# lazear/sage

Hardware: AMD Instinct MI355X
Metric: spectra/sec (whole node), fragment-index search-and-score, human tryptic narrow search (higher is better)
Workload: dtype f32

## Files before the change

include/sage_hip.h:

```cpp
#ifndef SAGE_HIP_H
#define SAGE_HIP_H

#include <stddef.h>
#include <stdint.h>

#ifdef __cplusplus
extern "C" {
#endif

#define SAGE_HIP_ABI_VERSION 6

enum {
    SAGE_HIP_OK = 0,
    SAGE_HIP_ERR_INVALID = 1,
    SAGE_HIP_ERR_NO_DEVICE = 2,
    SAGE_HIP_ERR_HIP = 3,
    SAGE_HIP_ERR_UNSUPPORTED = 4,
    SAGE_HIP_ERR_OOM = 5,
    SAGE_HIP_ERR_INTERNAL = 6
};

enum { SAGE_TOL_PPM = 0, SAGE_TOL_PCT = 1, SAGE_TOL_DA = 2 };
typedef struct SageTolerance {
    int32_t kind;
// ... 182 lines not shown
    float retry_ms;
    uint32_t n_tied;
    uint32_t n_ways;
} SageTiming;
int sage_hip_last_timing(const SageScorer* scorer, SageTiming* out);
int sage_hip_scorer_set_timing_interval(SageScorer* scorer, uint32_t every);

int sage_hip_host_alloc(uint64_t bytes, void** out);
void sage_hip_host_free(void* p);

int sage_hip_debug_phase_cycles(SageScorer* scorer, unsigned long long* out32);
int sage_hip_debug_prune_counters(SageScorer* scorer, unsigned long long* out4);
int sage_hip_debug_filter_counters(SageScorer* scorer, unsigned long long* out4);
int sage_hip_debug_heavy_counters(SageScorer* scorer, unsigned long long* out2);
int sage_hip_debug_heavy_routes(SageScorer* scorer, unsigned long long* out2);
int sage_hip_debug_handover_route(SageScorer* scorer, uint32_t* out);
#define SAGE_HIP_RESCORE_INST_CHIMERA 1u
#define SAGE_HIP_RESCORE_INST_KINDS2 2u
#define SAGE_HIP_RESCORE_INST_FAST 4u
#define SAGE_HIP_RESCORE_INST_ACC 8u
#define SAGE_HIP_RESCORE_INST_PROF 16u
#define SAGE_HIP_RESCORE_INST_BIG 32u
#define SAGE_HIP_RESCORE_INST_NONE 0xFFFFFFFFu
int sage_hip_debug_rescore_instance(SageScorer* scorer, uint32_t* out);

typedef struct SageDbLayout {
    uint64_t np, nf;
    uint32_t tile_shift, n_tiles, lut_stride;
    float lut_scale;
    uint32_t tile2_shift, n_tiles2, lut2_stride;
// ... 309 lines not shown
```

sage_amd/_lib.py:

```python
import ctypes as C
import os

import numpy as np

from . import build as _build

c_float_p = C.POINTER(C.c_float)
c_u8_p = C.POINTER(C.c_uint8)
c_u32_p = C.POINTER(C.c_uint32)
c_u64_p = C.POINTER(C.c_uint64)


class SageTolerance(C.Structure):
    _fields_ = [("kind", C.c_int32), ("lo", C.c_float), ("hi", C.c_float)]


class SageTheoretical(C.Structure):
    _fields_ = [("peptide_index", C.c_uint32), ("fragment_mz", C.c_float)]


class SageDbParams(C.Structure):
    _fields_ = [
        ("bucket_size", C.c_uint64),
        ("missed_cleavages", C.c_int32),
# ... 311 lines not shown
        "sage_hip_batch_upload_kinds": (C.c_int, [vp, C.POINTER(SageSpectrumBatch), c_u8_p, C.POINTER(vp)]),
        "sage_hip_batch_process_upload_kinds": (C.c_int, [vp, C.POINTER(SageRawBatch), c_u8_p, C.c_uint64, C.c_int, C.c_float,
                                                          C.c_uint32, C.POINTER(vp), c_u32_p]),
        "sage_hip_score_batch_kinds": (C.c_int, [vp, C.POINTER(SageSpectrumBatch), c_u8_p, vp, c_u32_p]),
        "sage_hip_score_resident": (C.c_int, [vp, vp, vp, c_u32_p]),
        "sage_hip_initial_hits": (C.c_int, [vp, vp, c_u64_p, C.c_uint32, c_u32_p, c_u64_p, c_u64_p]),
        "sage_hip_last_timing": (C.c_int, [vp, C.POINTER(SageTiming)]),
        "sage_hip_scorer_set_timing_interval": (C.c_int, [vp, C.c_uint32]),
        "sage_hip_annotate_resident": (C.c_int, [vp, vp, vp, c_u32_p, C.POINTER(SageFragments)]),
        "sage_hip_quick_score_resident": (C.c_int, [vp, vp, C.c_int, c_u8_p]),
        "sage_hip_debug_phase_cycles": (C.c_int, [vp, c_u64_p]),
        "sage_hip_debug_prune_counters": (C.c_int, [vp, c_u64_p]),
        "sage_hip_debug_filter_counters": (C.c_int, [vp, c_u64_p]),
        "sage_hip_debug_heavy_counters": (C.c_int, [vp, c_u64_p]),
        "sage_hip_debug_heavy_routes": (C.c_int, [vp, c_u64_p]),
        "sage_hip_debug_handover_route": (C.c_int, [vp, c_u32_p]),
        "sage_hip_debug_rescore_instance": (C.c_int, [vp, c_u32_p]),
        "sage_hip_debug_db_layout": (C.c_int, [vp, C.POINTER(SageDbLayout)]),
        "sage_hip_debug_db_table": (C.c_int, [vp, C.c_int, vp, C.c_uint64, c_u64_p]),
        "sage_hip_host_alloc": (C.c_int, [C.c_uint64, C.POINTER(vp)]),
        "sage_hip_host_free": (None, [vp]),
        "sage_hip_rescore": (C.c_int, [C.c_int, C.POINTER(SageRescoreInput), C.POINTER(SageRescoreOutput)]),
        "sage_hip_hostdb_competition_keys": (C.c_int, [vp, c_u32_p, C.c_uint64, c_u32_p, c_u32_p, c_u32_p, c_u32_p]),
        "sage_hip_predict_rt": (C.c_int, [C.c_int, C.POINTER(SageRtInput), C.POINTER(SageRtOutput)]),
        "sage_hip_hostdb_feature_peptides": (C.c_int, [vp, c_u32_p, C.c_uint64, c_u64_p, c_u8_p, c_float_p]),
        "sage_hip_mzml_read": (C.c_int, [C.c_char_p, C.c_uint32, C.c_int, C.POINTER(vp)]),
        "sage_hip_mzml_view": (C.c_int, [vp, C.POINTER(SageRawBatch)]),
        "sage_hip_mzml_check_searchable": (C.c_int, [vp]),
        "sage_hip_mzml_spectrum_id": (C.c_char_p, [vp, C.c_uint64]),
        "sage_hip_mzml_free": (None, [vp]),
# ... 39 lines not shown
    }
    for name, (res, args) in sig.items():
        fn = getattr(lib, name)
        fn.restype = res
        fn.argtypes = args
    _lib = lib
    return lib


EXPORTED_SYMBOLS = [
    "sage_hip_last_error", "sage_hip_abi_version", "sage_hip_hostdb_build", "sage_hip_hostdb_free",
    "sage_hip_hostdb_view", "sage_hip_hostdb_peptide_string", "sage_hip_hostdb_peptide_proteins",
    "sage_hip_hostdb_peptide_info", "sage_hip_process_ms2", "sage_hip_device_count", "sage_hip_db_create", "sage_hip_db_destroy",
    "sage_hip_db_device_bytes", "sage_hip_scorer_create", "sage_hip_scorer_destroy", "sage_hip_scorer_clone", "sage_hip_score_batch",
    "sage_hip_batch_upload", "sage_hip_batch_free", "sage_hip_batch_process_upload", "sage_hip_batch_download", "sage_hip_score_resident", "sage_hip_initial_hits",
    "sage_hip_last_timing", "sage_hip_scorer_set_timing_interval", "sage_hip_annotate_resident", "sage_hip_quick_score_resident", "sage_hip_debug_phase_cycles", "sage_hip_debug_prune_counters", "sage_hip_debug_filter_counters", "sage_hip_debug_heavy_counters", "sage_hip_debug_heavy_routes", "sage_hip_debug_handover_route", "sage_hip_debug_rescore_instance", "sage_hip_debug_db_layout", "sage_hip_debug_db_table", "sage_hip_host_alloc", "sage_hip_host_free",
    "sage_hip_rescore", "sage_hip_hostdb_competition_keys", "sage_hip_fasta_num_targets", "sage_hip_prefilter_chunk_size",
    "sage_hip_hostdb_build_chunk", "sage_hip_hostdb_merge_kept", "sage_hip_predict_rt", "sage_hip_hostdb_feature_peptides",
    "sage_hip_write_results", "sage_hip_mzml_read", "sage_hip_mzml_view", "sage_hip_mzml_check_searchable", "sage_hip_mzml_spectrum_id", "sage_hip_mzml_free",
    "sage_hip_lfq", "sage_hip_write_lfq", "sage_hip_mzml_read_sn", "sage_hip_mzml_ion_injection_time", "sage_hip_mzml_precursor_ref",
    "sage_hip_tmt", "sage_hip_write_tmt", "sage_hip_mgf_read", "sage_hip_mzml_isolation_kinds", "sage_hip_mzml_charge_zero",
    "sage_hip_parse_f32", "sage_hip_batch_upload_kinds", "sage_hip_batch_process_upload_kinds", "sage_hip_score_batch_kinds",
    "sage_hip_lfq_im", "sage_hip_mzml_mobility", "sage_hip_mzml_has_mobility",
    "sage_hip_protein_groups", "sage_hip_group_string", "sage_hip_group_strings_free", "sage_hip_group_graph_build",
    "sage_hip_group_graph_view", "sage_hip_group_graph_free", "sage_hip_hostdb_protein_name", "sage_hip_write_results_grouped",
    "sage_hip_hostdb_isomer_groups", "sage_hip_score_candidates_resident", "sage_hip_last_candidates_timing",
    "sage_hip_localise_resident", "sage_hip_ascore_from_counts", "sage_hip_last_localise_timing",
]


def check(rc):
# ... 8 lines not shown
```

sage_amd/csrc/capi.hip:

```cpp
#include <hip/hip_runtime.h>
#include <algorithm>
#include <atomic>
#include <cmath>
#include <chrono>
#include <cstring>
#include <memory>
#include <future>
#include <mutex>
#include <string>
#include <vector>

#include "crlog.h"
#include "device_types.h"
#define HIP_FAILED(e, what) fail(status_of(e), std::string(what) + ": " + hipGetErrorString(e))
#include "hip_host.h"
#include "host_db.hpp"

using namespace sagehip;

namespace {

thread_local std::string g_last_error;

int fail(int code, const std::string& msg) {
// ... 944 lines not shown
    d.list_cap = d.kmax * (std::max(n_iso, n_z) + 1);
    d.wcap = 1024;
    d.dbg_flags = 0;
    if (const char* e = getenv("SAGE_HIP_DEBUG_FLAGS")) d.dbg_flags = (uint32_t)atoi(e);
    s->hand_rows = (d.dbg_flags & 131072u) == 0u;
    d.prune_min = (d.dbg_flags & 4096u) ? 0u : d.min_matched_peaks;
    d.rescore_general = 0;
    if (const char* e = getenv("SAGE_HIP_RESCORE_GENERAL")) d.rescore_general = atoi(e) != 0 ? RESCORE_GENERAL_CHIMERA : 0u;
    {
        const DevDbView& v = db->view;
        bool kinds2 = v.n_kinds == 2u && v.ion_kinds[0] <= 2 && v.ion_kinds[1] > 2;
        if (const char* e = getenv("SAGE_HIP_RESCORE_KINDS_GENERAL")) kinds2 = kinds2 && atoi(e) == 0;
        if (!kinds2) d.rescore_general |= RESCORE_GENERAL_KINDS;
    }
    d.exact = 0;
    d.xcd_chunk = 1024;
    if (const char* e = getenv("SAGE_HIP_XCD_CHUNK")) d.xcd_chunk = (uint32_t)std::max(0, atoi(e));
    {
        const char* e = getenv("SAGE_HIP_SCHED_DESC");
        if (!e || atoi(e)) d.xcd_chunk |= 0x80000000u;
        s->sched_desc_forced = e != nullptr;
    }
    if (const char* e = getenv("SAGE_HIP_EXACT")) s->exact_always = atoi(e) != 0;
    if (const char* e = getenv("SAGE_HIP_FUSED")) s->fused = atoi(e) != 0;
    if (const char* e = getenv("SAGE_HIP_ONE_LANE")) s->two_lanes = atoi(e) == 0;
    if (const char* e = getenv("SAGE_HIP_SEARCH_LAG")) s->search_lag = (uint32_t)std::max(0, atoi(e));
    if (const char* e = getenv("SAGE_HIP_REPLAY_WAVE_MAX")) s->replay_split = (uint64_t)atoll(e) & 0xFFFFFFFFull;
    if (const char* e = getenv("SAGE_HIP_REPLAY_LANE_MAX")) s->replay_split |= (uint64_t)(uint32_t)atoll(e) << 32;
    if (const char* e = getenv("SAGE_HIP_ONE_LAUNCH")) s->one_launch = atoi(e) != 0;
#ifndef SAGE_HIP_EXPERIMENTS
    if (s->one_launch || s->fused || getenv("SAGE_HIP_SEARCH_LAG"))
        return fail(SAGE_HIP_ERR_UNSUPPORTED, "SAGE_HIP_ONE_LAUNCH / SAGE_HIP_FUSED / SAGE_HIP_SEARCH_LAG need a build with -DSAGE_HIP_EXPERIMENTS");
#endif
    if (const char* e = getenv("SAGE_HIP_NO_ZEROCOPY")) s->zero_copy = atoi(e) == 0;
    if (const char* e = getenv("SAGE_HIP_NO_FAST_TIES")) s->fast_ties = atoi(e) == 0;
// ... 613 lines not shown
    w.tile_shift = s->db->view.tile_shift;
    w.dbg = s->dbg.p;
    return w;
}

enum { MODE_SCORE = 0,
       MODE_EXACT = 1,
       MODE_FAST = 2 };

static int enqueue_compute(SageScorer* s, const DevBatchView& view_in, OutSet& o, bool with_rescore, int mode, hipStream_t st,
                           SageFeature* rec = nullptr, bool wide = true, uint32_t list_off = 0, uint32_t* count_buf = nullptr,
                           int lane = 0, int phase = 0, uint32_t widest = 0xFFFFFFFFu) {
    if (lane && wide) return fail(SAGE_HIP_ERR_INTERNAL, "large windows on the second working set");
    WorkSet& wset = lane ? s->ws2 : s->ws;
    DevScorer sc = s->dev;
    if (wide && !s->sched_desc_forced) sc.xcd_chunk &= 0x7FFFFFFFu;
    DevBatchView view = view_in;
    {
        const WindowKey mine = window_key(s);
        view.sched_win = view.sched && view.sched_stride == SCHED_RECORD_WINDOW && view.sched_key && std::memcmp(view.sched_key, &mine, sizeof mine) == 0;
    }
    if (!view.probe && (size_t)view.fzcap * view.pcap * 8 > 48 * 1024) view.probe = 1;
    if (!view.probe) {
        const int rc_pm = ensure_pm_frag(s->db);
        if (rc_pm != SAGE_HIP_OK) return rc_pm;
    }
    const bool production = mode == MODE_SCORE && with_rescore;
    const bool fused = s->fused && production;
    if (!production) wide = true;
    int rc = ensure_work(s, view.n, lane, wide, st);
    if (rc != SAGE_HIP_OK) return rc;
// ... 990 lines not shown
        for (uint32_t k = 0; k < 2; k++) out2[k] += all[b * DBG_PRUNE_WORDS + 8 + k];
    return SAGE_HIP_OK;
}

int sage_hip_debug_heavy_routes(SageScorer* s, unsigned long long* out2) {
    if (!s || !out2) return fail(SAGE_HIP_ERR_INVALID, "null argument");
    if (!s->dbg.p) return fail(SAGE_HIP_ERR_INVALID, "set SAGE_HIP_PHASE_CLOCKS=1 before creating the scorer");
    std::vector<unsigned long long> all((size_t)DBG_BLOCKS * DBG_PRUNE_WORDS);
    HIP_TRY(hipMemcpy(all.data(), s->dbg.p + (size_t)DBG_BLOCKS * 32, all.size() * 8, hipMemcpyDeviceToHost));
    out2[0] = out2[1] = 0;
    for (size_t b = 0; b < DBG_BLOCKS; b++)
        for (uint32_t k = 0; k < 2; k++) out2[k] += all[b * DBG_PRUNE_WORDS + 10 + k];
    return SAGE_HIP_OK;
}

int sage_hip_debug_handover_route(SageScorer* s, uint32_t* out) {
    if (!s || !out) return fail(SAGE_HIP_ERR_INVALID, "null argument");
    *out = s->last_hand ? 1u : 0u;
    return SAGE_HIP_OK;
}

int sage_hip_debug_rescore_instance(SageScorer* s, uint32_t* out) {
    if (!s || !out) return fail(SAGE_HIP_ERR_INVALID, "null argument");
    static_assert(RESCORE_INST_CHIMERA == SAGE_HIP_RESCORE_INST_CHIMERA && RESCORE_INST_KINDS2 == SAGE_HIP_RESCORE_INST_KINDS2 &&
                      RESCORE_INST_FAST == SAGE_HIP_RESCORE_INST_FAST && RESCORE_INST_ACC == SAGE_HIP_RESCORE_INST_ACC &&
                      RESCORE_INST_PROF == SAGE_HIP_RESCORE_INST_PROF && RESCORE_INST_BIG == SAGE_HIP_RESCORE_INST_BIG &&
                      RESCORE_INST_NONE == SAGE_HIP_RESCORE_INST_NONE,
                  "include/sage_hip.h names the bits of device_types.h");
    *out = s->last_rescore;
    return SAGE_HIP_OK;
// ... 114 lines not shown
```

sage_amd/csrc/core.h:

```cpp
#pragma once
#include <stdint.h>

#if defined(__HIPCC__)
#define SAGE_HD __host__ __device__ __forceinline__
#else
#define SAGE_HD inline
#endif

namespace sagecore {

constexpr float PROTON = 1.0072764f;
constexpr float NEUTRON = 1.00335f;

struct Tol {
    int kind;
    float lo, hi;
};

SAGE_HD void tol_bounds(const Tol& t, float center, float& out_lo, float& out_hi) {
    if (t.kind == 0) {
        float dlo = center * t.lo / 1000000.0f;
        float dhi = center * t.hi / 1000000.0f;
        out_lo = center + dlo;
        out_hi = center + dhi;
// ... 640 lines not shown
#ifndef SAGE_FLAT_MARGIN
#define SAGE_FLAT_MARGIN 1
#endif
constexpr uint32_t FLAT_MARGIN = SAGE_FLAT_MARGIN;
SAGE_HD uint32_t flat_route_bar(uint32_t total) { return (total + 63u) / 64u + FLAT_MARGIN; }
SAGE_HD bool flat_route_wins(uint32_t total, uint32_t longest) { return total != 0u && longest > flat_route_bar(total); }
SAGE_HD uint32_t flat_mask_word(uint32_t lo, uint32_t hi, uint32_t start) {
#if defined(__HIP_DEVICE_COMPILE__)
    return __builtin_amdgcn_alignbyte(hi, lo, start & 3u);
#else
    const uint32_t sh = (start & 3u) * 8u;
    return sh ? (lo >> sh) | (hi << (32u - sh)) : lo;
#endif
}

}
```

sage_amd/csrc/device_types.h:

```cpp
#pragma once
#include <stdint.h>

#include <string>

#include "../../include/sage_hip.h"
#include "core.h"

namespace sagehip {

struct DevDbView {
    const float* pep_mono;
    uint32_t np;
    const uint32_t* pep_lut;
    uint32_t pep_lut_bins;
    float pep_lut_inv_w;
    const SageTheoretical* pm_frag;
    const uint64_t* pm_off;
    const float* ions;
    const uint64_t* ion_off;
    const uint32_t* pep_info;
    const SageTheoretical* tm_frag;
    const uint32_t* tm_lut;
    uint32_t tile_shift;
    uint32_t n_tiles;
// ... 3 lines not shown
    const sagecore::LutWord* tm2_l1;
    const uint32_t* tm2_pos;
    uint32_t lut2_words;
    uint32_t tile2_shift;
    uint32_t n_tiles2;
    uint32_t lut2_stride;
    float lut2_scale;
    uint64_t nf;
    uint8_t ion_kinds[8];
    uint32_t n_kinds;
};

constexpr uint32_t TILE_SHIFT_MAX = 15;
__host__ __device__ inline size_t tm_lut_index(uint32_t t, uint32_t c, uint32_t lut_stride) { return (size_t)t * lut_stride + c; }

constexpr uint32_t DBG_BLOCKS = 4096, DBG_PRUNE_WORDS = 12;
constexpr size_t DBG_TOTAL_WORDS = (size_t)DBG_BLOCKS * (32 + DBG_PRUNE_WORDS);

struct DevScorer {
    sagecore::Tol precursor_tol, fragment_tol;
    sagecore::PbmReach pbm_reach;
    uint32_t min_matched_peaks;
    int min_isotope_err, max_isotope_err;
    uint32_t min_precursor_charge, max_precursor_charge;
    uint32_t override_precursor_charge;
    int max_fragment_charge;
    uint32_t chimera;
    uint32_t report_psms;
    uint32_t wide_window;
    int score_type;
    uint32_t kmax;
// ... 213 lines not shown
```

sage_amd/csrc/kernels.hip:

```cpp
#include <hip/hip_runtime.h>

#include <type_traits>

#include "crlog.h"
#include "device_types.h"

using namespace sagecore;

namespace sagehip {

namespace {

#ifndef SAGE_PRELIM_WAVES
#define SAGE_PRELIM_WAVES 5
#endif
#ifndef SAGE_RESCORE_WAVES
#define SAGE_RESCORE_WAVES 5
#endif
#ifndef SAGE_NARROW_WAVES
#define SAGE_NARROW_WAVES 5
#endif
#ifndef SAGE_PROBE_PER_LANE
#define SAGE_PROBE_PER_LANE 2
#endif
// ... 9 lines not shown
#ifndef SAGE_MARK_BLOCKS16
#define SAGE_MARK_BLOCKS16 40
#endif
#ifndef SAGE_COOP_MIN_HITS
#define SAGE_COOP_MIN_HITS 12
#endif
#ifndef SAGE_COOP_MAX_LANES
#define SAGE_COOP_MAX_LANES 2
#endif
#ifndef SAGE_CNT_MODE
#define SAGE_CNT_MODE 0
#endif
#ifndef SAGE_SCAN_SKIP
#define SAGE_SCAN_SKIP 1
#endif
#if SAGE_NARROW_WAVES
#define SAGE_NARROW_WAVES_ATTR __attribute__((amdgpu_waves_per_eu(SAGE_NARROW_WAVES, SAGE_NARROW_WAVES)))
#else
#define SAGE_NARROW_WAVES_ATTR
#endif
#if SAGE_PRELIM_WAVES
#define SAGE_PRELIM_WAVES_ATTR __attribute__((amdgpu_waves_per_eu(SAGE_PRELIM_WAVES, SAGE_PRELIM_WAVES)))
#else
#define SAGE_PRELIM_WAVES_ATTR
#endif
#if SAGE_RESCORE_WAVES
#define SAGE_RESCORE_WAVES_ATTR __attribute__((amdgpu_waves_per_eu(SAGE_RESCORE_WAVES, SAGE_RESCORE_WAVES)))
#else
#define SAGE_RESCORE_WAVES_ATTR
#endif

constexpr uint32_t WAVE = 64;
constexpr uint32_t NO_WINDOW = 0xFFFFFFFFu;
constexpr uint32_t FAST_TIE_WORDS = PBM_WORDS + PLUT_BINS;
constexpr uint32_t CNT_ROW_HEADER = 4;
constexpr uint32_t PROBE_BATCH_WORDS = SAGE_PROBE_PER_LANE * 64;
constexpr uint32_t PROBE_TCS_WORDS = PROBE_BATCH_WORDS <= 64 ? 64 : PROBE_BATCH_WORDS <= 128 ? 128 : PROBE_BATCH_WORDS <= 256 ? 256 : 512;
constexpr uint32_t PROBE_TABLE_WORDS = 4 * PROBE_BATCH_WORDS + PROBE_TCS_WORDS;

enum { DBG_PRUNE_CAND = 0, DBG_PRUNE_ITEMS = 1, DBG_PRUNE_EARLY = 2, DBG_PRUNE_MIXED = 3 };
enum { DBG_FILTER_FLAT_CHUNKS = 4, DBG_FILTER_FLAT_TRIPS = 5, DBG_FILTER_FLAT_WOULD = 6, DBG_FILTER_LANE_TRIPS = 7 };
enum { DBG_HEAVY_CHUNKS = 8, DBG_HEAVY_ITEMS = 9 };
enum { DBG_HEAVY_ONE_TRIP = 10, DBG_HEAVY_PER_CHARGE = 11 };
enum { DBG_NARROW_LUT = 26, DBG_NARROW_CELLS = 27, DBG_RESCORE = 28, DBG_TILE_LUT = 29, DBG_TILE_CELLS = 30, DBG_TILE_CAND = 31 };
struct PhaseClock {
    unsigned long long* slot;
    long long t;
    __device__ __forceinline__ void bytes(int which, unsigned long long n) {
        if (slot) atomicAdd(&slot[which - row_base], n);
    }
    int row_base;
    unsigned long long* prune;
    uint32_t pruned_here;
    __device__ __forceinline__ void pruned(uint64_t lanes, uint32_t items) {
        if (slot && lanes) {
            pruned_here += (uint32_t)__popcll(lanes);
            if ((threadIdx.x & 63u) == 0) {
                atomicAdd(&prune[DBG_PRUNE_CAND], (unsigned long long)__popcll(lanes));
// ... 9 lines not shown
                atomicAdd(&prune[DBG_FILTER_FLAT_WOULD], (unsigned long long)lane_trips);
            } else {
                atomicAdd(&prune[DBG_FILTER_LANE_TRIPS], (unsigned long long)lane_trips);
            }
        }
    }
    __device__ __forceinline__ void heavy(uint32_t items) {
        if (slot && (threadIdx.x & 63u) == 0) {
            atomicAdd(&prune[DBG_HEAVY_CHUNKS], 1ull);
            atomicAdd(&prune[DBG_HEAVY_ITEMS], (unsigned long long)items);
        }
    }
    __device__ __forceinline__ void heavy_route(bool one_trip) {
        if (slot && (threadIdx.x & 63u) == 0) atomicAdd(&prune[one_trip ? DBG_HEAVY_ONE_TRIP : DBG_HEAVY_PER_CHARGE], 1ull);
    }
    __device__ __forceinline__ void prune_outcome(bool left_early, bool any_pass) {
        if (slot && (threadIdx.x & 63u) == 0) {
            if (left_early) atomicAdd(&prune[DBG_PRUNE_EARLY], 1ull);
            else if (any_pass && pruned_here) atomicAdd(&prune[DBG_PRUNE_MIXED], 1ull);
        }
        pruned_here = 0;
    }
    __device__ __forceinline__ void start(unsigned long long* dbg, uint32_t blk, uint32_t kernel) {
        slot = dbg ? dbg + (size_t)(blk % DBG_BLOCKS) * 32 + kernel * 8 : nullptr;
        row_base = (int)kernel * 8;
        prune = dbg ? dbg + (size_t)DBG_BLOCKS * 32 + (size_t)(blk % DBG_BLOCKS) * DBG_PRUNE_WORDS : nullptr;
        pruned_here = 0;
        if (slot) t = clock64();
    }
    __device__ __forceinline__ void mark(int phase) {
// ... 5 lines not shown
    }
    __device__ __forceinline__ void rebase(uint32_t kernel) {
        if (slot) slot += (int)kernel * 8 - row_base;
        row_base = (int)kernel * 8;
    }
};

struct NoClock {
    static constexpr unsigned long long* slot = nullptr;
    __device__ __forceinline__ void bytes(int, unsigned long long) {}
    __device__ __forceinline__ void pruned(uint64_t, uint32_t) {}
    __device__ __forceinline__ void prune_outcome(bool, bool) {}
    __device__ __forceinline__ void filter_trips(bool, uint32_t, uint32_t) {}
    __device__ __forceinline__ void heavy(uint32_t) {}
    __device__ __forceinline__ void heavy_route(bool) {}
    __device__ __forceinline__ void start(unsigned long long*, uint32_t, uint32_t) {}
    __device__ __forceinline__ void mark(int) {}
    __device__ __forceinline__ void rebase(uint32_t) {}
};

__device__ __forceinline__ uint32_t lane_id() { return threadIdx.x & 63u; }

constexpr uint32_t N_XCD = 8;
__device__ __forceinline__ uint32_t xcd_position_fwd(uint32_t b, uint32_t n, uint32_t chunk) {
    if (chunk == 0) return b;
    const uint32_t group = N_XCD * chunk;
    if (b >= n / group * group) return b;
    const uint32_t x = b % N_XCD, i = b / N_XCD;
    return ((i / chunk) * N_XCD + x) * chunk + i % chunk;
}
__device__ __forceinline__ uint32_t xcd_position(uint32_t b, uint32_t n, uint32_t chunk) {
    const uint32_t p = xcd_position_fwd(b, n, chunk & 0x7FFFFFFFu);
    return (chunk & 0x80000000u) ? n - 1 - p : p;
}

__device__ __forceinline__ uint32_t fresh_zero() {
    uint32_t z;
    asm volatile("v_mov_b32 %0, 0" : "=v"(z));
    return z;
}
__device__ __forceinline__ uint32_t uni(uint32_t v) { return (uint32_t)__builtin_amdgcn_readfirstlane((int)v); }
__device__ __forceinline__ float unif(float v) { return __int_as_float(__builtin_amdgcn_readfirstlane(__float_as_int(v))); }
__device__ __forceinline__ uint64_t uni64(uint64_t v) { return ((uint64_t)uni((uint32_t)(v >> 32)) << 32) | uni((uint32_t)v); }

__device__ __forceinline__ uint32_t wave_sum_dpp(uint32_t v) {
    v += (uint32_t)__builtin_amdgcn_update_dpp(0, (int)v, 0xb1, 0xf, 0xf, false);
    v += (uint32_t)__builtin_amdgcn_update_dpp(0, (int)v, 0x4e, 0xf, 0xf, false);
    v += (uint32_t)__builtin_amdgcn_update_dpp(0, (int)v, 0x124, 0xf, 0xf, false);
    v += (uint32_t)__builtin_amdgcn_update_dpp(0, (int)v, 0x128, 0xf, 0xf, false);
// ... 373 lines not shown
    s.mzp = unif(b.precursor_mz[spec]) - PROTON;
    s.iso_tol.kind = 2;
    s.iso_tol.lo = -2.4f;
    s.iso_tol.hi = 2.4f;
    if (b.isolation_lo && b.isolation_hi) {
        const float a = unif(b.isolation_lo[spec]), c = unif(b.isolation_hi[spec]);
        if (a == a && c == c) {
            s.iso_tol.lo = a;
            s.iso_tol.hi = c;
            if (b.iso_kind) s.iso_tol.kind = (int32_t)uni(b.iso_kind[spec]);
        }
    }
    return s;
}

__device__ __forceinline__ SpecInfo load_spec_sched(const DevScorer& sc, const DevBatchView& b, uint32_t pos, uint32_t& spec) {
    const uint4* __restrict__ rec = b.sched + (size_t)b.sched_stride * pos;
    const uint4 r0 = rec[0], r1 = rec[1];
    uint4 r2 = make_uint4(NO_WINDOW, 0u, 0u, 0u);
    if (b.sched_win) r2 = rec[2];
    spec = uni(r0.x);
    SpecInfo s;
    s.win = Window{uni(r2.x), uni(r2.y), uni(r2.z), uni(r2.w)};
    s.has_win = s.win.left != NO_WINDOW;
    s.p0 = ((uint64_t)uni(r0.w) << 32) | uni(r0.z);
    s.P = uni(r0.y);
    const uint32_t zraw = uni(r1.x) & 0xFFu;
    if (sc.wide_window || zraw == 0 || sc.override_precursor_charge) {
        s.z0 = sc.min_precursor_charge;
        s.z1 = sc.max_precursor_charge;
    } else {
        s.z0 = s.z1 = zraw;
    }
    s.nfz_max = 0;
    for (uint32_t z = s.z0; z <= s.z1; z++) {
        const uint32_t m = max_fragment_charge(sc.max_fragment_charge, z) - 1;
        s.nfz_max = m > s.nfz_max ? m : s.nfz_max;
    }
    if (s.nfz_max > b.fzcap) s.nfz_max = b.fzcap;
    s.mzp = unif(__uint_as_float(r1.y)) - PROTON;
    s.iso_tol.kind = 2;
    s.iso_tol.lo = -2.4f;
    s.iso_tol.hi = 2.4f;
    const float a = unif(__uint_as_float(r1.z)), c = unif(__uint_as_float(r1.w));
    if (a == a && c == c) {
        s.iso_tol.lo = a;
        s.iso_tol.hi = c;
        s.iso_tol.kind = (int32_t)(((uni(r1.x) >> 8) & 0xFFu) ^ 2u);
    }
    return s;
}

template <bool GALLOP>
__device__ __forceinline__ Window query_window(const float* __restrict__ pep_mono, const uint32_t np, const Tol& ptol, float center,
                                               const uint32_t* __restrict__ lut = nullptr, const uint32_t bins = 0, const float inv_w = 0.0f) {
    float plo, phi;
    tol_bounds(ptol, center, plo, phi);
    Window q;
    uint32_t left, right;
    if (lut && plo >= 0.0f && phi >= plo && phi * inv_w < (float)bins) {
        const uint32_t b0 = uni((uint32_t)(plo * inv_w)), b1 = uni((uint32_t)(phi * inv_w));
        const uint32_t l0 = lut[b0], l1 = lut[b0 + 1], r0 = lut[b1], r1 = lut[b1 + 1];
        if (l1 - l0 < WAVE && r1 - r0 < WAVE) {
            const uint32_t lane = lane_id();
            const uint32_t base_l = l0 ? l0 - 1 : 0;
// ... 25 lines not shown
                ghi = (uint64_t)left + span < np ? (uint32_t)(left + span) : np;
                if (ghi == np || order_key(pep_mono[ghi - 1]) > order_key(phi)) break;
            }
        }
        right = wave_partition_point<false>(pep_mono, left, ghi, order_key(phi));
    }
    q.left = left;
    q.right = right;
    q.first = left;
    q.end = right;
    if (left < np && !(pep_mono[left] >= plo)) q.first = left + 1;
    if (right < np && pep_mono[right] <= phi) q.end = right + 1;
    return q;
}

__device__ __forceinline__ bool fast_select(const PrelimLds& L, const Counters& cnt, uint32_t potential, uint32_t k, uint32_t left,
                                            uint32_t z, int iso, uint32_t kmax, UList& target, uint32_t& scored) {
    const uint32_t lane = lane_id();
    uint32_t* hist = (uint32_t*)L.heap;
    wave_sync();
    hist[lane] = 0;
    wave_sync();
    for (uint32_t base = 0; base < potential; base += WAVE) {
        const uint32_t i = base + lane;
        const uint32_t c = i < potential ? cnt.get(i) : 0;
        if (c) atomicAdd(&hist[c < 63 ? c : 63], 1u);
    }
    wave_sync();
    const uint32_t mine = hist[lane];
    const uint32_t incl_pre = wave_incl_scan_dpp(mine);
    const uint32_t suffix = (uint32_t)__builtin_amdgcn_readlane((int)incl_pre, 63) - incl_pre + mine;
    if (__builtin_amdgcn_readlane((int)mine, 63) != 0) return false;
    scored = (uint32_t)__builtin_amdgcn_readlane((int)suffix, 1);
    const uint64_t okm = __ballot(lane >= 1 && suffix >= k);
    const uint32_t T = uni(okm ? 63u - (uint32_t)__clzll((long long)okm) : 0u);
    const uint32_t n_gt = (uint32_t)__builtin_amdgcn_readlane((int)suffix, (int)(T + 1 < 64 ? T + 1 : 63));
    const uint32_t n_eq = T ? (uint32_t)__builtin_amdgcn_readlane((int)mine, (int)T) : 0;
    const uint32_t take_eq = T ? k - n_gt : 0, skip_eq = n_eq - take_eq;
    wave_sync();
    uint64_t* sel = L.heap;
    uint32_t nsel = 0, eq_seen = 0;
    for (uint32_t base = 0; base < potential; base += WAVE) {
        const uint32_t i = base + lane;
        const uint32_t c = i < potential ? cnt.get(i) : 0;
        const uint64_t eqm = __ballot(T != 0 && c == T);
        const uint32_t eq_idx = eq_seen + (uint32_t)__popcll(eqm & ((1ull << lane) - 1ull));
        const bool take = c > T || (T != 0 && c == T && eq_idx >= skip_eq);
        const uint64_t tm = __ballot(take);
        if (take) sel[nsel + (uint32_t)__popcll(tm & ((1ull << lane) - 1ull))] = pack_prescore(c, left + i, z, iso);
        nsel += (uint32_t)__popcll(tm);
        eq_seen += (uint32_t)__popcll(eqm);
    }
    wave_sync();
    ulist_append(target, lane < nsel ? sel[lane] : PRESCORE_EMPTY, k, kmax);
    wave_sync();
    return true;
}

constexpr uint32_t PROBE_PER_LANE = SAGE_PROBE_PER_LANE;
constexpr uint32_t PROBE_BATCH = PROBE_PER_LANE * 64;
constexpr uint32_t PROBE_CELLS = SAGE_PROBE_CELLS;
static_assert(PROBE_BATCH == PROBE_BATCH_WORDS && PROBE_BATCH <= 512, "the run table's layout (carve_prelim) is the kernel's");
static_assert(PROBE_TCS_WORDS - PROBE_BATCH <= WAVE, "one sentinel per lane pads the run starts");
struct PrelimKernargs {
// ... 340 lines not shown
                    for (uint32_t base = 0; base < k; base += WAVE) {
                        const uint32_t i = base + lane;
                        const uint32_t c = i < k ? cnt.get(i) : 0;
                        if (i < k) hp[i] = c ? pack_prescore(c, left + i, z, iso) : PRESCORE_EMPTY;
                        scored += (uint32_t)__popcll(__ballot(c > 0));
                    }
                    lh_build(hp, k);
                    for (uint32_t base = k; base < potential; base += WAVE) {
                        const uint32_t i = base + lane;
                        const uint32_t c = i < potential ? cnt.get(i) : 0;
                        scored += (uint32_t)__popcll(__ballot(c > 0));
                        lh_offer_batch(hp, k, pack_prescore(c, left + i, z, iso), c > 0);
                    }
                    for (uint32_t base = 0; base < k; base += WAVE)
                        ulist_append(target, base + lane < k ? hp[base + lane] : PRESCORE_EMPTY, k - base < WAVE ? k - base : WAVE, kmax);
                } else if (!exact && fast_select(L, cnt, potential, k, left, z, iso, kmax, target, scored)) {
                    res.untrimmed = false;
                } else {
                    res.untrimmed = false;
                    scored = 0;
                    Heap32 hp;
                    {
                        const uint32_t c = lane < k ? cnt.get(lane) : 0;
                        wh32_init(hp, c ? (c << 16) | lane : 0u, k);
                        scored += (uint32_t)__popcll(__ballot(c > 0));
                    }
                    wh32_build(hp, k);
                    for (uint32_t base = k; base < potential; base += WAVE) {
                        const uint32_t i = base + lane;
                        const uint32_t c = i < potential ? cnt.get(i) : 0;
                        const uint32_t v = (c << 16) | i;
// ... 43 lines not shown
        res.scored = tot_scored;
        res.ok = A.ok && B.ok;
    }
    return res;
}

template <bool PROBE, bool PROF, bool BIGK = false, bool HUGE = false>
__global__ __launch_bounds__(64) SAGE_PRELIM_WAVES_ATTR void prelim_kernel(PrelimKernargs A) {
    const DevDbView& db = A.db;
    const DevScorer& sc = A.sc;
    const DevBatchView& b = A.b;
    const DevWork& w = A.w;
    typedef typename std::conditional<PROF, PhaseClock, NoClock>::type Clock;
    extern __shared__ __align__(16) unsigned char smem[];
    const uint32_t lane = lane_id();
    const PrelimLds L = carve_prelim(smem, sc, b, BIGK && HUGE ? w.hugebuf + (size_t)blockIdx.x * w.huge_stride : nullptr);

    uint32_t n_batch = b.n;
    if (b.n_dev) {
        const uint32_t nd = uni(*b.n_dev);
        n_batch = nd < n_batch ? nd : n_batch;
    }
    for (uint32_t blk = blockIdx.x; blk < n_batch; blk += gridDim.x) {
        const uint32_t pos = xcd_position(blk, n_batch, sc.xcd_chunk);
        uint32_t spec = b.sched ? 0u : b.order ? uni(b.order[pos]) : pos;
        __syncthreads();
        Clock pc;
        pc.start((sc.dbg_flags & 512u) && !sc.exact ? nullptr : w.dbg, blk, 0);
        const SpecInfo si = b.sched ? load_spec_sched(sc, b, pos, spec) : load_spec(sc, b, spec);
        const PrelimResult r = prelim_spectrum<PROBE, BIGK, PrelimKernargs>(db, sc, b, L, si, sc.exact != 0, pc);
        typedef const __attribute__((address_space(4))) PrelimKernargs* Segment;
        Segment ka = (Segment)__builtin_amdgcn_kernarg_segment_ptr();
        asm volatile("" : "+s"(ka));
        uint32_t* const w_cnt_store = ka->w.cnt_store;
        if (!BIGK && w_cnt_store) {
            const bool keep = !r.deferred && si.z0 == si.z1 && ka->sc.min_isotope_err == ka->sc.max_isotope_err;
            uint32_t* __restrict__ row = w_cnt_store + (size_t)pos * ka->w.cnt_stride;
            if (keep && SAGE_CNT_MODE != 1)
                for (uint32_t i = lane; i < (r.q_potential + 1) / 2; i += WAVE) row[CNT_ROW_HEADER + i] = L.cnt[i];
            if (lane == 0 && SAGE_CNT_MODE != 2) {
                row[0] = keep ? r.q_left : 0u;
                row[1] = keep ? r.q_potential : 0u;
            }
        }
// ... 3 lines not shown
            const uint32_t stored = r.deferred ? 0u : (r.stored < HAND_LIST_MAX ? r.stored : HAND_LIST_MAX);
            uint64_t v = lane < stored ? L.listB[lane] : PRESCORE_EMPTY;
            if (lane == HAND_HEAD_WORD) v = (uint64_t)stored << 32 | st;
            if (lane == HAND_TOTALS_WORD) v = r.deferred ? 0ull : (uint64_t)r.scored << 32 | r.matched;
            w_hand[(size_t)pos * HAND_ROW_WORDS + lane] = v;
        }
        if (r.deferred) {
            if (lane == 0) {
                ka->w.status[spec] = ST_DEFERRED;
                if (!ka->w.queue_later) {
                    const uint32_t it = atomicAdd(ka->w.n_deferred + CTR_QUEUED, 1u);
                    ka->w.queue[it] = spec;
                    if (!ka->w.reuse) ka->w.item_of[spec] = it;
                }
            }
            continue;
        }
        if (lane == 0 && !r.ok) atomicAdd(ka->w.n_deferred + CTR_LIST_OVERFLOW, 1u);
        if (!w_hand) {
            if (lane == 0) {
                ka->w.status[spec] = r.ok ? (r.untrimmed ? ST_OK_ORDERED : ST_OK) : ST_OVERFLOW;
                ka->w.cand_len[spec] = r.stored;
                ka->w.totals[2 * spec] = r.matched;
                ka->w.totals[2 * spec + 1] = r.scored;
            }
            uint64_t* __restrict__ dst = ka->w.cand + (size_t)spec * ka->sc.kmax;
            for (uint32_t i = lane; i < r.stored; i += WAVE) dst[i] = L.listB[i];
        }
        pc.mark(4);
    }
}

__global__ __launch_bounds__(256) void queue_kernel(DevScorer sc, DevBatchView b, DevWork w) {
    uint32_t n_batch = b.n;
    if (b.n_dev) {
        const uint32_t nd = *b.n_dev;
        n_batch = nd < n_batch ? nd : n_batch;
    }
    const uint32_t lane = lane_id();
    for (uint32_t base = blockIdx.x * blockDim.x; base < n_batch; base += gridDim.x * blockDim.x) {
        const uint32_t blk = base + threadIdx.x;
        uint32_t spec = 0;
        bool marked = false;
        if (blk < n_batch) {
// ... 3286 lines not shown
```

Baseline: 162.8 million.

## Prefetch next schedule record, add one-pass top-k select, shift-based XCD mapping

```diff
diff --git a/include/sage_hip.h b/include/sage_hip.h
--- a/include/sage_hip.h
+++ b/include/sage_hip.h
@@ -220,6 +220,7 @@
 int sage_hip_debug_filter_counters(SageScorer* scorer, unsigned long long* out4);
 int sage_hip_debug_heavy_counters(SageScorer* scorer, unsigned long long* out2);
 int sage_hip_debug_heavy_routes(SageScorer* scorer, unsigned long long* out2);
+int sage_hip_debug_select_routes(SageScorer* scorer, unsigned long long* out2);
 int sage_hip_debug_handover_route(SageScorer* scorer, uint32_t* out);
 #define SAGE_HIP_RESCORE_INST_CHIMERA 1u
 #define SAGE_HIP_RESCORE_INST_KINDS2 2u
diff --git a/sage_amd/_lib.py b/sage_amd/_lib.py
--- a/sage_amd/_lib.py
+++ b/sage_amd/_lib.py
@@ -349,6 +349,7 @@
         "sage_hip_debug_filter_counters": (C.c_int, [vp, c_u64_p]),
         "sage_hip_debug_heavy_counters": (C.c_int, [vp, c_u64_p]),
         "sage_hip_debug_heavy_routes": (C.c_int, [vp, c_u64_p]),
+        "sage_hip_debug_select_routes": (C.c_int, [vp, c_u64_p]),
         "sage_hip_debug_handover_route": (C.c_int, [vp, c_u32_p]),
         "sage_hip_debug_rescore_instance": (C.c_int, [vp, c_u32_p]),
         "sage_hip_debug_db_layout": (C.c_int, [vp, C.POINTER(SageDbLayout)]),
@@ -418,7 +419,7 @@
     "sage_hip_hostdb_peptide_info", "sage_hip_process_ms2", "sage_hip_device_count", "sage_hip_db_create", "sage_hip_db_destroy",
     "sage_hip_db_device_bytes", "sage_hip_scorer_create", "sage_hip_scorer_destroy", "sage_hip_scorer_clone", "sage_hip_score_batch",
     "sage_hip_batch_upload", "sage_hip_batch_free", "sage_hip_batch_process_upload", "sage_hip_batch_download", "sage_hip_score_resident", "sage_hip_initial_hits",
-    "sage_hip_last_timing", "sage_hip_scorer_set_timing_interval", "sage_hip_annotate_resident", "sage_hip_quick_score_resident", "sage_hip_debug_phase_cycles", "sage_hip_debug_prune_counters", "sage_hip_debug_filter_counters", "sage_hip_debug_heavy_counters", "sage_hip_debug_heavy_routes", "sage_hip_debug_handover_route", "sage_hip_debug_rescore_instance", "sage_hip_debug_db_layout", "sage_hip_debug_db_table", "sage_hip_host_alloc", "sage_hip_host_free",
+    "sage_hip_last_timing", "sage_hip_scorer_set_timing_interval", "sage_hip_annotate_resident", "sage_hip_quick_score_resident", "sage_hip_debug_phase_cycles", "sage_hip_debug_prune_counters", "sage_hip_debug_filter_counters", "sage_hip_debug_heavy_counters", "sage_hip_debug_heavy_routes", "sage_hip_debug_select_routes", "sage_hip_debug_handover_route", "sage_hip_debug_rescore_instance", "sage_hip_debug_db_layout", "sage_hip_debug_db_table", "sage_hip_host_alloc", "sage_hip_host_free",
     "sage_hip_rescore", "sage_hip_hostdb_competition_keys", "sage_hip_fasta_num_targets", "sage_hip_prefilter_chunk_size",
     "sage_hip_hostdb_build_chunk", "sage_hip_hostdb_merge_kept", "sage_hip_predict_rt", "sage_hip_hostdb_feature_peptides",
     "sage_hip_write_results", "sage_hip_mzml_read", "sage_hip_mzml_view", "sage_hip_mzml_check_searchable", "sage_hip_mzml_spectrum_id", "sage_hip_mzml_free",
diff --git a/sage_amd/csrc/capi.hip b/sage_amd/csrc/capi.hip
--- a/sage_amd/csrc/capi.hip
+++ b/sage_amd/csrc/capi.hip
@@ -982,11 +982,11 @@
         if (!kinds2) d.rescore_general |= RESCORE_GENERAL_KINDS;
     }
     d.exact = 0;
-    d.xcd_chunk = 1024;
-    if (const char* e = getenv("SAGE_HIP_XCD_CHUNK")) d.xcd_chunk = (uint32_t)std::max(0, atoi(e));
+    uint32_t xcd_chunk = 1024;
+    if (const char* e = getenv("SAGE_HIP_XCD_CHUNK")) xcd_chunk = (uint32_t)std::max(0, atoi(e));
     {
         const char* e = getenv("SAGE_HIP_SCHED_DESC");
-        if (!e || atoi(e)) d.xcd_chunk |= 0x80000000u;
+        d.xcd_chunk = sagecore::xcd_chunk_word(xcd_chunk, !e || atoi(e), (d.dbg_flags & 1048576u) != 0u);
         s->sched_desc_forced = e != nullptr;
     }
     if (const char* e = getenv("SAGE_HIP_EXACT")) s->exact_always = atoi(e) != 0;
@@ -1630,7 +1630,7 @@
     if (lane && wide) return fail(SAGE_HIP_ERR_INTERNAL, "large windows on the second working set");
     WorkSet& wset = lane ? s->ws2 : s->ws;
     DevScorer sc = s->dev;
-    if (wide && !s->sched_desc_forced) sc.xcd_chunk &= 0x7FFFFFFFu;
+    if (wide && !s->sched_desc_forced) sc.xcd_chunk &= ~sagecore::XCD_CHUNK_DESC;
     DevBatchView view = view_in;
     {
         const WindowKey mine = window_key(s);
@@ -2651,6 +2651,17 @@
     return SAGE_HIP_OK;
 }
 
+int sage_hip_debug_select_routes(SageScorer* s, unsigned long long* out2) {
+    if (!s || !out2) return fail(SAGE_HIP_ERR_INVALID, "null argument");
+    if (!s->dbg.p) return fail(SAGE_HIP_ERR_INVALID, "set SAGE_HIP_PHASE_CLOCKS=1 before creating the scorer");
+    std::vector<unsigned long long> all((size_t)DBG_BLOCKS * DBG_PRUNE_WORDS);
+    HIP_TRY(hipMemcpy(all.data(), s->dbg.p + (size_t)DBG_BLOCKS * 32, all.size() * 8, hipMemcpyDeviceToHost));
+    out2[0] = out2[1] = 0;
+    for (size_t b = 0; b < DBG_BLOCKS; b++)
+        for (uint32_t k = 0; k < 2; k++) out2[k] += all[b * DBG_PRUNE_WORDS + 12 + k];
+    return SAGE_HIP_OK;
+}
+
 int sage_hip_debug_handover_route(SageScorer* s, uint32_t* out) {
     if (!s || !out) return fail(SAGE_HIP_ERR_INVALID, "null argument");
     *out = s->last_hand ? 1u : 0u;
diff --git a/sage_amd/csrc/core.h b/sage_amd/csrc/core.h
--- a/sage_amd/csrc/core.h
+++ b/sage_amd/csrc/core.h
@@ -678,4 +678,40 @@
 #endif
 }
 
-}
+constexpr uint32_t N_XCD = 8;
+constexpr uint32_t XCD_CHUNK_DESC = 0x80000000u, XCD_CHUNK_POW2 = 0x40000000u, XCD_CHUNK_MAX = 0x0FFFFFFFu;
+SAGE_HD uint32_t xcd_position_fwd(uint32_t b, uint32_t n, uint32_t chunk) {
+    if (chunk == 0) return b;
+    const uint32_t group = N_XCD * chunk;
+    if (b >= n / group * group) return b;
+    const uint32_t x = b % N_XCD, i = b / N_XCD;
+    return ((i / chunk) * N_XCD + x) * chunk + i % chunk;
+}
+SAGE_HD uint32_t xcd_position_fwd_shift(uint32_t b, uint32_t n, uint32_t log2_chunk) {
+    const uint32_t group_mask = (N_XCD << log2_chunk) - 1u;
+    if (b >= (n & ~group_mask)) return b;
+    const uint32_t x = b & (N_XCD - 1u), i = b >> 3;
+    return ((((i >> log2_chunk) << 3) + x) << log2_chunk) + (i & ((1u << log2_chunk) - 1u));
+}
+SAGE_HD uint32_t xcd_position(uint32_t b, uint32_t n, uint32_t chunk_word) {
+    const uint32_t chunk = chunk_word & XCD_CHUNK_MAX;
+    const uint32_t p = (chunk_word & XCD_CHUNK_POW2) ? xcd_position_fwd_shift(b, n, (uint32_t)__builtin_ctz(chunk))
+                                                     : xcd_position_fwd(b, n, chunk);
+    return (chunk_word & XCD_CHUNK_DESC) ? n - 1 - p : p;
+}
+SAGE_HD uint32_t xcd_chunk_word(uint32_t chunk, bool desc, bool force_division) {
+    if (chunk > XCD_CHUNK_MAX) chunk = XCD_CHUNK_MAX;
+    const bool pow2 = chunk != 0 && (chunk & (chunk - 1u)) == 0;
+    return chunk | (pow2 && !force_division ? XCD_CHUNK_POW2 : 0u) | (desc ? XCD_CHUNK_DESC : 0u);
+}
+
+constexpr uint32_t SELECT_BINS = 64;
+SAGE_HD uint32_t select_bin(uint32_t c) { return c < SELECT_BINS - 1u ? c : SELECT_BINS - 1u; }
+SAGE_HD bool select_exact_only(uint32_t c) { return c >= SELECT_BINS - 1u; }
+SAGE_HD bool select_one_pass(uint32_t nonempty, uint32_t k) { return nonempty <= k; }
+SAGE_HD uint32_t select_threshold(uint64_t ok) { return ok ? 63u - (uint32_t)__builtin_clzll(ok) : 0u; }
+SAGE_HD bool select_take(uint32_t c, uint32_t T, uint32_t eq_idx, uint32_t skip_eq) {
+    return c > T || (T != 0 && c == T && eq_idx >= skip_eq);
+}
+
+}
diff --git a/sage_amd/csrc/device_types.h b/sage_amd/csrc/device_types.h
--- a/sage_amd/csrc/device_types.h
+++ b/sage_amd/csrc/device_types.h
@@ -41,7 +41,7 @@
 constexpr uint32_t TILE_SHIFT_MAX = 15;
 __host__ __device__ inline size_t tm_lut_index(uint32_t t, uint32_t c, uint32_t lut_stride) { return (size_t)t * lut_stride + c; }
 
-constexpr uint32_t DBG_BLOCKS = 4096, DBG_PRUNE_WORDS = 12;
+constexpr uint32_t DBG_BLOCKS = 4096, DBG_PRUNE_WORDS = 14;
 constexpr size_t DBG_TOTAL_WORDS = (size_t)DBG_BLOCKS * (32 + DBG_PRUNE_WORDS);
 
 struct DevScorer {
diff --git a/sage_amd/csrc/kernels.hip b/sage_amd/csrc/kernels.hip
--- a/sage_amd/csrc/kernels.hip
+++ b/sage_amd/csrc/kernels.hip
@@ -47,6 +47,12 @@
 #ifndef SAGE_SCAN_SKIP
 #define SAGE_SCAN_SKIP 1
 #endif
+#ifndef SAGE_SELECT_ONE_PASS
+#define SAGE_SELECT_ONE_PASS 1
+#endif
+#ifndef SAGE_RECORD_AHEAD
+#define SAGE_RECORD_AHEAD 1
+#endif
 #if SAGE_NARROW_WAVES
 #define SAGE_NARROW_WAVES_ATTR __attribute__((amdgpu_waves_per_eu(SAGE_NARROW_WAVES, SAGE_NARROW_WAVES)))
 #else
@@ -75,6 +81,7 @@
 enum { DBG_FILTER_FLAT_CHUNKS = 4, DBG_FILTER_FLAT_TRIPS = 5, DBG_FILTER_FLAT_WOULD = 6, DBG_FILTER_LANE_TRIPS = 7 };
 enum { DBG_HEAVY_CHUNKS = 8, DBG_HEAVY_ITEMS = 9 };
 enum { DBG_HEAVY_ONE_TRIP = 10, DBG_HEAVY_PER_CHARGE = 11 };
+enum { DBG_SELECT_ONE_PASS = 12, DBG_SELECT_THRESHOLD = 13 };
 enum { DBG_NARROW_LUT = 26, DBG_NARROW_CELLS = 27, DBG_RESCORE = 28, DBG_TILE_LUT = 29, DBG_TILE_CELLS = 30, DBG_TILE_CAND = 31 };
 struct PhaseClock {
     unsigned long long* slot;
@@ -114,6 +121,9 @@
     __device__ __forceinline__ void heavy_route(bool one_trip) {
         if (slot && (threadIdx.x & 63u) == 0) atomicAdd(&prune[one_trip ? DBG_HEAVY_ONE_TRIP : DBG_HEAVY_PER_CHARGE], 1ull);
     }
+    __device__ __forceinline__ void select_route(bool one_pass) {
+        if (slot && (threadIdx.x & 63u) == 0) atomicAdd(&prune[one_pass ? DBG_SELECT_ONE_PASS : DBG_SELECT_THRESHOLD], 1ull);
+    }
     __device__ __forceinline__ void prune_outcome(bool left_early, bool any_pass) {
         if (slot && (threadIdx.x & 63u) == 0) {
             if (left_early) atomicAdd(&prune[DBG_PRUNE_EARLY], 1ull);
@@ -149,6 +159,7 @@
     __device__ __forceinline__ void filter_trips(bool, uint32_t, uint32_t) {}
     __device__ __forceinline__ void heavy(uint32_t) {}
     __device__ __forceinline__ void heavy_route(bool) {}
+    __device__ __forceinline__ void select_route(bool) {}
     __device__ __forceinline__ void start(unsigned long long*, uint32_t, uint32_t) {}
     __device__ __forceinline__ void mark(int) {}
     __device__ __forceinline__ void rebase(uint32_t) {}
@@ -156,18 +167,6 @@
 
 __device__ __forceinline__ uint32_t lane_id() { return threadIdx.x & 63u; }
 
-constexpr uint32_t N_XCD = 8;
-__device__ __forceinline__ uint32_t xcd_position_fwd(uint32_t b, uint32_t n, uint32_t chunk) {
-    if (chunk == 0) return b;
-    const uint32_t group = N_XCD * chunk;
-    if (b >= n / group * group) return b;
-    const uint32_t x = b % N_XCD, i = b / N_XCD;
-    return ((i / chunk) * N_XCD + x) * chunk + i % chunk;
-}
-__device__ __forceinline__ uint32_t xcd_position(uint32_t b, uint32_t n, uint32_t chunk) {
-    const uint32_t p = xcd_position_fwd(b, n, chunk & 0x7FFFFFFFu);
-    return (chunk & 0x80000000u) ? n - 1 - p : p;
-}
 
 __device__ __forceinline__ uint32_t fresh_zero() {
     uint32_t z;
@@ -571,11 +570,20 @@
     return s;
 }
 
-__device__ __forceinline__ SpecInfo load_spec_sched(const DevScorer& sc, const DevBatchView& b, uint32_t pos, uint32_t& spec) {
-    const uint4* __restrict__ rec = b.sched + (size_t)b.sched_stride * pos;
-    const uint4 r0 = rec[0], r1 = rec[1];
-    uint4 r2 = make_uint4(NO_WINDOW, 0u, 0u, 0u);
-    if (b.sched_win) r2 = rec[2];
+__device__ __forceinline__ void sched_request(const uint4* __restrict__ sched, uint32_t stride, uint32_t with_window, uint32_t pos, uint4& r0,
+                                              uint4& r1, uint4& r2) {
+    const uint4* __restrict__ rec = sched + (size_t)stride * pos;
+    r0 = rec[0];
+    r1 = rec[1];
+    r2 = make_uint4(NO_WINDOW, 0u, 0u, 0u);
+    if (with_window) r2 = rec[2];
+}
+template <class B>
+__device__ __forceinline__ void sched_request(const B& b, uint32_t pos, uint4& r0, uint4& r1, uint4& r2) {
+    sched_request(b.sched, b.sched_stride, b.sched_win, pos, r0, r1, r2);
+}
+__device__ __forceinline__ SpecInfo spec_of_record(const DevScorer& sc, const DevBatchView& b, const uint4 r0, const uint4 r1, const uint4 r2,
+                                                   uint32_t& spec) {
     spec = uni(r0.x);
     SpecInfo s;
     s.win = Window{uni(r2.x), uni(r2.y), uni(r2.z), uni(r2.w)};
@@ -606,6 +614,12 @@
         s.iso_tol.kind = (int32_t)(((uni(r1.x) >> 8) & 0xFFu) ^ 2u);
     }
     return s;
+}
+
+__device__ __forceinline__ SpecInfo load_spec_sched(const DevScorer& sc, const DevBatchView& b, uint32_t pos, uint32_t& spec) {
+    uint4 r0, r1, r2;
+    sched_request(b, pos, r0, r1, r2);
+    return spec_of_record(sc, b, r0, r1, r2, spec);
 }
 
 template <bool GALLOP>
@@ -661,9 +675,37 @@
     return q;
 }
 
+template <class PC>
 __device__ __forceinline__ bool fast_select(const PrelimLds& L, const Counters& cnt, uint32_t potential, uint32_t k, uint32_t left,
-                                            uint32_t z, int iso, uint32_t kmax, UList& target, uint32_t& scored) {
+                                            uint32_t z, int iso, uint32_t kmax, UList& target, uint32_t& scored, const bool force_threshold,
+                                            PC& pc) {
     const uint32_t lane = lane_id();
+    const uint64_t below = (1ull << lane) - 1ull;
+    uint64_t* sel = L.heap;
+    wave_sync();
+    if (SAGE_SELECT_ONE_PASS) {
+        uint32_t nz = 0;
+        uint64_t too_big = 0ull;
+        for (uint32_t base = 0; base < potential; base += WAVE) {
+            const uint32_t i = base + lane;
+            const uint32_t c = i < potential ? cnt.get(i) : 0;
+            const uint64_t m = __ballot(c != 0);
+            too_big |= __ballot(select_exact_only(c));
+            const uint32_t at = nz + (uint32_t)__popcll(m & below);
+            if (c && at < k) sel[at] = pack_prescore(c, left + i, z, iso);
+            nz += (uint32_t)__popcll(m);
+            if (!select_one_pass(nz, k)) break;
+        }
+        if (select_one_pass(nz, k) && too_big) return false;
+        if (select_one_pass(nz, k) && !force_threshold) {
+            pc.select_route(true);
+            scored = nz;
+            wave_sync();
+            ulist_append(target, lane < nz ? sel[lane] : PRESCORE_EMPTY, k, kmax);
+            wave_sync();
+            return true;
+        }
+    }
     uint32_t* hist = (uint32_t*)L.heap;
     wave_sync();
     hist[lane] = 0;
@@ -671,30 +713,30 @@
     for (uint32_t base = 0; base < potential; base += WAVE) {
         const uint32_t i = base + lane;
         const uint32_t c = i < potential ? cnt.get(i) : 0;
-        if (c) atomicAdd(&hist[c < 63 ? c : 63], 1u);
+        if (c) atomicAdd(&hist[select_bin(c)], 1u);
     }
     wave_sync();
     const uint32_t mine = hist[lane];
     const uint32_t incl_pre = wave_incl_scan_dpp(mine);
     const uint32_t suffix = (uint32_t)__builtin_amdgcn_readlane((int)incl_pre, 63) - incl_pre + mine;
     if (__builtin_amdgcn_readlane((int)mine, 63) != 0) return false;
+    pc.select_route(false);
     scored = (uint32_t)__builtin_amdgcn_readlane((int)suffix, 1);
     const uint64_t okm = __ballot(lane >= 1 && suffix >= k);
-    const uint32_t T = uni(okm ? 63u - (uint32_t)__clzll((long long)okm) : 0u);
+    const uint32_t T = uni(select_threshold(okm));
     const uint32_t n_gt = (uint32_t)__builtin_amdgcn_readlane((int)suffix, (int)(T + 1 < 64 ? T + 1 : 63));
     const uint32_t n_eq = T ? (uint32_t)__builtin_amdgcn_readlane((int)mine, (int)T) : 0;
     const uint32_t take_eq = T ? k - n_gt : 0, skip_eq = n_eq - take_eq;
     wave_sync();
-    uint64_t* sel = L.heap;
     uint32_t nsel = 0, eq_seen = 0;
     for (uint32_t base = 0; base < potential; base += WAVE) {
         const uint32_t i = base + lane;
         const uint32_t c = i < potential ? cnt.get(i) : 0;
         const uint64_t eqm = __ballot(T != 0 && c == T);
-        const uint32_t eq_idx = eq_seen + (uint32_t)__popcll(eqm & ((1ull << lane) - 1ull));
-        const bool take = c > T || (T != 0 && c == T && eq_idx >= skip_eq);
+        const uint32_t eq_idx = eq_seen + (uint32_t)__popcll(eqm & below);
+        const bool take = select_take(c, T, eq_idx, skip_eq);
         const uint64_t tm = __ballot(take);
-        if (take) sel[nsel + (uint32_t)__popcll(tm & ((1ull << lane) - 1ull))] = pack_prescore(c, left + i, z, iso);
+        if (take) sel[nsel + (uint32_t)__popcll(tm & below)] = pack_prescore(c, left + i, z, iso);
         nsel += (uint32_t)__popcll(tm);
         eq_seen += (uint32_t)__popcll(eqm);
     }
@@ -1065,7 +1107,7 @@
                     }
                     for (uint32_t base = 0; base < k; base += WAVE)
                         ulist_append(target, base + lane < k ? hp[base + lane] : PRESCORE_EMPTY, k - base < WAVE ? k - base : WAVE, kmax);
-                } else if (!exact && fast_select(L, cnt, potential, k, left, z, iso, kmax, target, scored)) {
+                } else if (!exact && fast_select(L, cnt, potential, k, left, z, iso, kmax, target, scored, (av.sc().dbg_flags & 524288u) != 0u, pc)) {
                     res.untrimmed = false;
                 } else {
                     res.untrimmed = false;
@@ -1139,6 +1181,23 @@
     typedef typename std::conditional<PROF, PhaseClock, NoClock>::type Clock;
     extern __shared__ __align__(16) unsigned char smem[];
     const uint32_t lane = lane_id();
+    uint4 rec0 = make_uint4(0u, 0u, 0u, 0u), rec1 = rec0, rec2 = make_uint4(NO_WINDOW, 0u, 0u, 0u);
+    bool ahead = false;
+    uint32_t pos = 0;
+    if (SAGE_RECORD_AHEAD) {
+        typedef const __attribute__((address_space(4))) PrelimKernargs* Segment;
+        Segment ka = (Segment)__builtin_amdgcn_kernarg_segment_ptr();
+        asm volatile("" : "+s"(ka));
+        const uint4* const k_sched = ka->b.sched;
+        const uint32_t* const k_n_dev = ka->b.n_dev;
+        const uint32_t k_n = ka->b.n, k_chunk = ka->sc.xcd_chunk, k_stride = ka->b.sched_stride, k_win = ka->b.sched_win;
+        asm volatile("" ::"s"(k_sched), "s"(k_n_dev), "s"(k_n), "s"(k_chunk), "s"(k_stride), "s"(k_win));
+        ahead = k_sched != nullptr && k_n_dev == nullptr;
+        if (ahead && blockIdx.x < k_n) {
+            pos = xcd_position(blockIdx.x, k_n, k_chunk);
+            sched_request(k_sched, k_stride, k_win, pos, rec0, rec1, rec2);
+        }
+    }
     const PrelimLds L = carve_prelim(smem, sc, b, BIGK && HUGE ? w.hugebuf + (size_t)blockIdx.x * w.huge_stride : nullptr);
 
     uint32_t n_batch = b.n;
@@ -1146,13 +1205,17 @@
         const uint32_t nd = uni(*b.n_dev);
         n_batch = nd < n_batch ? nd : n_batch;
     }
+    if (!ahead && blockIdx.x < n_batch) {
+        pos = xcd_position(blockIdx.x, n_batch, sc.xcd_chunk);
+        if (b.sched) sched_request(b, pos, rec0, rec1, rec2);
+    }
     for (uint32_t blk = blockIdx.x; blk < n_batch; blk += gridDim.x) {
-        const uint32_t pos = xcd_position(blk, n_batch, sc.xcd_chunk);
         uint32_t spec = b.sched ? 0u : b.order ? uni(b.order[pos]) : pos;
         __syncthreads();
         Clock pc;
         pc.start((sc.dbg_flags & 512u) && !sc.exact ? nullptr : w.dbg, blk, 0);
-        const SpecInfo si = b.sched ? load_spec_sched(sc, b, pos, spec) : load_spec(sc, b, spec);
+        const SpecInfo si = b.sched ? spec_of_record(sc, b, rec0, rec1, rec2, spec) : load_spec(sc, b, spec);
+        const uint32_t blk_next = blk + gridDim.x;
         const PrelimResult r = prelim_spectrum<PROBE, BIGK, PrelimKernargs>(db, sc, b, L, si, sc.exact != 0, pc);
         typedef const __attribute__((address_space(4))) PrelimKernargs* Segment;
         Segment ka = (Segment)__builtin_amdgcn_kernarg_segment_ptr();
@@ -1186,6 +1249,14 @@
                     if (!ka->w.reuse) ka->w.item_of[spec] = it;
                 }
             }
+            {
+                rec0 = rec1 = make_uint4(0u, 0u, 0u, 0u);
+                rec2 = make_uint4(NO_WINDOW, 0u, 0u, 0u);
+                if (blk_next < n_batch) {
+                    pos = xcd_position(blk_next, n_batch, ka->sc.xcd_chunk);
+                    if (ka->b.sched) sched_request(ka->b, pos, rec0, rec1, rec2);
+                }
+            }
             continue;
         }
         if (lane == 0 && !r.ok) atomicAdd(ka->w.n_deferred + CTR_LIST_OVERFLOW, 1u);
@@ -1200,6 +1271,14 @@
             for (uint32_t i = lane; i < r.stored; i += WAVE) dst[i] = L.listB[i];
         }
         pc.mark(4);
+        {
+                rec0 = rec1 = make_uint4(0u, 0u, 0u, 0u);
+                rec2 = make_uint4(NO_WINDOW, 0u, 0u, 0u);
+                if (blk_next < n_batch) {
+                    pos = xcd_position(blk_next, n_batch, ka->sc.xcd_chunk);
+                    if (ka->b.sched) sched_request(ka->b, pos, rec0, rec1, rec2);
+                }
+            }
     }
 }
 
```

New measurement: 163.4 million (median of 6 runs). No clear change (+0.3%).
